# sksundaram-learning/linkerd

Measured on AMD Instinct MI355X. Metric: histogram samples ingested+summarized/sec (1M series) and % HBM peak, higher is better.
Workload: dtype u32; 1 GPU; C3: 1M series, 1e9 Zipf(s=1) samples per step, log-normal values; series_total=1000000, series_per_gpu=1000000, rotating_batches=3, parallelism=series-sharded x1 (weighted ranges), step=ingest (sample+plan+bin1+bin2) + snapshot(reset, dense counts + summaries)

## Files before the change

### linkerd_amd/csrc/l5dh_ingest.hip

```cpp
#include <algorithm>
#include <type_traits>

#include "l5dh_device.hpp"

namespace l5dh {
namespace {

constexpr uint32_t RSAMPLE = 1u << 18;
#ifndef L5DH_RS_WG
#define L5DH_RS_WG 64
#endif
constexpr int RS_WG = L5DH_RS_WG;
static_assert((RSAMPLE + RS_WG - 1) / RS_WG <= 65535, "k_rsample's u16 LDS counters: at most 65535 draws per workgroup");
constexpr uint32_t INVALID = 0xFFFFFFFFu;

__device__ __forceinline__ uint32_t round_up(uint32_t x, uint32_t m) { return (x + m - 1) / m * m; }

__device__ __forceinline__ uint32_t rcap(double prev, double e, double s, bool exact, double pad, uint32_t align,
                                         uint32_t pct, double z, bool floor_sample) {
  double c;
  if (exact) {
    c = e;
  } else {
    const double e0 = prev / s, sg = sqrt(e0 + 1.0);
    const double r = sqrt(e + 1.0) + 0.5 * z;
    const double sb = !floor_sample && prev == 0.0 && e == 0.0 ? ceil(4.0 * s) : ceil(r * r * s);
    if (prev > 0.0 && e >= e0 - 6.0 * sg && (floor_sample || e <= e0 + 4.0 * sg)) {
      c = ceil(prev * 1.0625 + 4.0 * sqrt(prev));
      if (floor_sample) c = fmax(c, sb);
    } else {
      c = sb;
    }
    c += pad;
  }
  if (pct != 100) c = floor(c * (double)pct / 100.0);
  return round_up((uint32_t)fmin(c, 1073741824.0), align);
}

__device__ __forceinline__ uint64_t block_excl_scan64(uint64_t v, uint64_t* lds , uint64_t* total) {
  const int lane = threadIdx.x & 63, w = threadIdx.x >> 6;
  const uint64_t incl = wave_incl_scan(v);
  if (lane == 63) lds[w] = incl;
  __syncthreads();
  if (threadIdx.x == 0) {
    uint64_t acc = 0;
    for (int k = 0; k < 16; ++k) {
      const uint64_t q = lds[k];
      lds[k] = acc;
      acc += q;
    }
    lds[16] = acc;
  }
  __syncthreads();
  const uint64_t r = lds[w] + incl - v;
  *total = lds[16];
  __syncthreads();
  return r;
}

#ifdef L5DH_PHASES
__device__ unsigned long long g_phase_plan[16];
#define RP_MARK(k) \
  if (threadIdx.x == 0) g_phase_plan[k] = wall_clock64();
#define RS_MARK(k) \
  if (threadIdx.x == 0 && blockIdx.x == 0) g_phase_plan[k] = wall_clock64();
#else
#define RP_MARK(k)
#define RS_MARK(k)
#endif

__global__ __launch_bounds__(1024) void k_rsample(const uint32_t* __restrict__ series, size_t n, uint32_t S, uint32_t K,
                                                  uint32_t* __restrict__ kest) {
  extern __shared__ uint32_t c[];
  RS_MARK(8)
  for (uint32_t i = threadIdx.x; i < (K + 1) / 2; i += 1024) c[i] = 0;
  __syncthreads();
  RS_MARK(9)
  const uint64_t m = n < RSAMPLE ? n : RSAMPLE;
  const uint64_t per = (m + RS_WG - 1) / RS_WG;
  const uint64_t k0 = blockIdx.x * per, k1 = k0 + per < m ? k0 + per : m;
  for (uint64_t kb = k0; kb < k1; kb += 4 * 1024) {
    uint32_t sv[4];
#pragma unroll
    for (int u = 0; u < 4; ++u) {
      const uint64_t k = kb + threadIdx.x + 1024u * u;
      const uint64_t i = m == n ? k : k * n / m;
      sv[u] = k < k1 ? series[i < n ? i : 0] : 0xFFFFFFFFu;
    }
#pragma unroll
    for (int u = 0; u < 4; ++u)
      if (sv[u] < S) {
        const uint32_t key = sv[u] >> 4;
        atomicAdd(&c[key >> 1], (key & 1u) ? 0x10000u : 1u);
      }
  }
  __syncthreads();
  RS_MARK(10)
  for (uint32_t i = threadIdx.x; i < (K + 1) / 2; i += 1024) {
    const uint32_t x = c[i];
    if (x & 0xFFFFu) atomicAdd(&kest[2 * i], x & 0xFFFFu);
    if ((x >> 16) && 2 * i + 1 < K) atomicAdd(&kest[2 * i + 1], x >> 16);
  }
  RS_MARK(11)
}

constexpr size_t RPLAN1_LDS = 32768 * 4;
constexpr uint32_t RFIX2_ONE_WG_MAX = 16384;
__global__ __launch_bounds__(1024) void k_rplan1(size_t n, uint32_t F, const uint32_t* __restrict__ kest,
                                                 const uint32_t* __restrict__ kprev, uint32_t* __restrict__ meta,
                                                 size_t cap32, size_t dlim16, uint32_t thr_min, uint32_t dmax,
                                                 uint32_t pct) {
  __shared__ uint32_t lh[33];
  __shared__ uint32_t sthr;
  __shared__ uint4 lds4[17];
  __shared__ uint64_t l64[17];
  __shared__ uint32_t dl[DIRECT_MAX + 1];
  __shared__ uint32_t capl[BIN1_BINS];
  extern __shared__ uint32_t tw[];
  const MetaLayout L = meta_layout(F);
  const uint32_t FS = (F + ST_TILES - 1) / ST_TILES;
  const uint32_t NW = (F + 31) / 32;
  const uint64_t m = n < RSAMPLE ? n : RSAMPLE;
  const bool exact = m == n;
  const double s = m ? (double)n / (double)m : 1.0;
  const uint32_t j = threadIdx.x, t0 = j * 32;
  const int lane = lane_id();
  RP_MARK(0)
  if (j < 33) lh[j] = 0;
  capl[j] = 0;
  auto load_pairs = [&](const uint32_t* __restrict__ kw, uint4 (&x)[16]) {
#pragma unroll
    for (int i = 0; i < 16; ++i) {
      const uint32_t t = 2u * (j + 1024u * (uint32_t)i);
      x[i] = make_uint4(0u, 0u, 0u, 0u);
      if (t + 1 < F) {
        x[i] = *reinterpret_cast<const uint4*>(kw + 2 * t);
      } else if (t < F) {
        x[i].x = kw[2 * t];
        x[i].y = kw[2 * t + 1];
      }
    }
  };
  uint2 te[16];
  {
    uint4 x[16];
    load_pairs(kest, x);
#pragma unroll
    for (int i = 0; i < 16; ++i) te[i] = make_uint2(x[i].x + x[i].y, x[i].z + x[i].w);
  }
  auto scaled = [&](uint32_t v) -> uint32_t { return (uint32_t)fmin((double)v * s, 4294967295.0); };
  __syncthreads();
  RP_MARK(1)
  auto hist = [&](uint32_t v) {
    const uint32_t e = scaled(v);
    const bool ok = dmax > 0 && e >= thr_min && e > 0;
    const int bin = ok ? 31 - __clz((int)e) : 0;
    const uint64_t act = __ballot(ok);
    if (!act) return;
    const int b0 = __builtin_amdgcn_readlane(bin, __builtin_ctzll(act));
    if (__ballot(ok && bin == b0) == act) {
      if (lane == 0) atomicAdd(&lh[b0], (uint32_t)__popcll(act));
    } else if (ok) {
      atomicAdd(&lh[bin], 1u);
    }
  };
#pragma unroll
  for (int i = 0; i < 16; ++i) {
    hist(te[i].x);
    hist(te[i].y);
  }
  __syncthreads();
  if (j < 64) {
    const uint32_t c = j < 32 ? lh[31 - j] : 0u;
    const uint32_t cum = wave_incl_scan32(c);
    const uint64_t ok = __ballot(dmax > 0 && j < 32 && cum <= dmax);
    const int nb = __popcll(ok);
    if (j == 0) sthr = nb ? max(max(thr_min, 1u), 1u << (32 - nb)) : 0xFFFFFFFFu;
  }
#pragma unroll
  for (int i = 0; i < 16; ++i) reinterpret_cast<uint2*>(tw)[j + 1024u * (uint32_t)i] = te[i];
  uint4 xp[16];
  load_pairs(kprev, xp);
  __syncthreads();
  const uint32_t thr = sthr;
  RP_MARK(2)
  uint32_t dbits = 0, E = 0;
#pragma unroll
  for (int k = 0; k < 32; ++k) {
    const uint32_t kk = (uint32_t)(k + (int)j) & 31u;
    const uint32_t v = tw[t0 + kk];
    if (t0 + kk < F && scaled(v) >= thr) dbits |= 1u << kk;
    else E += v;
  }
  __syncthreads();
#pragma unroll
  for (int i = 0; i < 16; ++i)
    reinterpret_cast<uint2*>(tw)[j + 1024u * (uint32_t)i] = make_uint2(xp[i].x + xp[i].y, xp[i].z + xp[i].w);
  __syncthreads();
  uint64_t P = 0;
#pragma unroll
  for (int k = 0; k < 32; ++k) {
    const uint32_t kk = (uint32_t)(k + (int)j) & 31u;
    if (!((dbits >> kk) & 1u)) P += tw[t0 + kk];
  }
  RP_MARK(3)
  uint32_t cv[4] = {(uint32_t)__popc(dbits), 0u, 0u, 0u}, ct[4];
  block_excl_scan4<1024>(cv, lds4, ct);
  const uint32_t ND = ct[0];
  meta[L.dbits() + j] = j < NW ? dbits : 0u;
  meta[L.dpre() + j] = cv[0];
  {
    uint32_t x = dbits, di = cv[0];
    while (x) {
      const uint32_t k = (uint32_t)(__ffs((int)x) - 1);
      x &= x - 1u;
      dl[di] = t0 + k;
      meta[L.dlist() + di] = t0 + k;
      ++di;
    }
  }
  P += __shfl_xor(P, 1, 64);
  E += __shfl_xor(E, 1, 64);
  RP_MARK(4)
  if ((j & 1u) == 0 && (j >> 1) < FS) {
    const uint32_t b = j >> 1;
    capl[b] = rcap((double)P, (double)E, s, exact, 256.0, 4, pct, 6.0, true);
    meta[L.btot() + b] = (uint32_t)min(P, (uint64_t)0xFFFFFFFFu);
  }
  __syncthreads();
  RP_MARK(5)
  const uint32_t TB = FS + 2 * ND;
  if (j >= FS && j < TB) {
    const uint32_t t = dl[(j - FS) >> 1], h = (j - FS) & 1u;
    const double p = (double)kprev[2 * t + h], e = (double)kest[2 * t + h];
    capl[j] = rcap(p, e, s, exact, 256.0, 8, pct, 5.0, false);
  }
  __syncthreads();
  const bool stb = j < FS, dj = j >= FS && j < TB;
  uint64_t tot32, tot16;
  const uint64_t base32 = block_excl_scan64(stb ? (uint64_t)capl[j] : 0ull, l64, &tot32);
  const uint64_t base16 = block_excl_scan64(dj ? (uint64_t)capl[j] : 0ull, l64, &tot16);
  const uint64_t base = stb ? base32 : base16;
  const uint64_t lim = stb ? cap32 : dlim16;
  if (base + capl[j] + 16 > lim)
    capl[j] = base + 16 < lim ? (uint32_t)(lim - 16 - base) & (stb ? ~3u : ~7u) : 0u;
  meta[L.bbase() + j] = (uint32_t)base;
  meta[L.bcap() + j] = j < TB ? capl[j] : 0u;
  meta[L.bcnt() + j] = 0u;
  if (j == 0) {
    uint32_t* hdr = meta + L.hdr();
    hdr[H_ND] = ND;
    hdr[H_OV1] = 0;
    hdr[H_REDO1] = 0;
    hdr[H_OV2] = 0;
    hdr[H_REDO2] = 0;
    hdr[H_COUNT2] = 0;
    hdr[H_EXACT] = exact ? 1u : 0u;
    hdr[H_D16] = (uint32_t)min(tot16, (uint64_t)dlim16);
  }
  RP_MARK(6)
}

#ifdef L5DH_PHASES
__device__ unsigned long long g_phase1[1024 * 8];
__device__ unsigned long long g_phase3[1024 * 8];
#define PH_INIT                                                            \
  const bool ph_on = threadIdx.x == 0 || threadIdx.x == NT1 - 64;          \
  uint32_t ph_acc[8] = {0, 0, 0, 0, 0, 0, 0, 0}, ph_t = (uint32_t)wall_clock64();
#define PH_VWAIT asm volatile("s_waitcnt vmcnt(0)" ::: "memory");
#define PH_MARK(k)                                 \
  if (ph_on) {                                     \
    const uint32_t ph_n = (uint32_t)wall_clock64(); \
    ph_acc[k] += ph_n - ph_t;                      \
    ph_t = ph_n;                                   \
  }
#define PH_FLUSH                                                                          \
  if (ph_on && pass == 0 && (threadIdx.x == 0 || gridDim.x <= 256)) {                      \
    const uint32_t ph_row = blockIdx.x + (threadIdx.x ? 512u : 0u);                       \
    for (int k = 0; k < 7; ++k) g_phase1[ph_row * 8 + k] += ph_acc[k];                    \
    g_phase1[ph_row * 8 + 7] += 1;                                                        \
    if (gridDim.x <= 256) {                                                               \
      g_phase1[(768 + blockIdx.x) * 8 + (threadIdx.x ? 1 : 0)] += ph_acc[7];              \
      if (threadIdx.x == 0) g_phase1[(768 + blockIdx.x) * 8 + 7] += 1;                    \
    }                                                                                     \
  }
#else
#define PH_INIT
#define PH_MARK(k)
#define PH_VWAIT
#define PH_FLUSH
#endif
__device__ __forceinline__ uint4 ld_stream(const uint32_t* p) { return *reinterpret_cast<const uint4*>(p); }
constexpr int CHW = 16384;
constexpr int NT1 = 1024;
constexpr int B1_PT = CHW / NT1;
constexpr int B1_PH = B1_PT / 2;
constexpr int B1_GS = 4;
constexpr int B1_HG = B1_PH / 4;
static_assert(B1_PH % 4 == 0 && B1_PH % B1_GS == 0 && B1_GS % 4 == 0, "halves of whole 16-B groups");
static_assert(NT1 == BIN1_BINS, "one bin per thread");
constexpr uint32_t DSUM_PMAX = 1u << 17;
static_assert(DSUM_PMAX == 1u << 17, "the ranking loop tests the bits of 2^17f, 0x48000000");
constexpr uint32_t NODEST = 0xFFFFFFFFu - (uint32_t)CHW;
constexpr int DSUM_N = DIRECT_MAX * TILE;

struct Bin1Lds {
  static constexpr int DW_N = 1024;
  static constexpr size_t o_stage = 0;
  static constexpr size_t o_cnt = o_stage + CHW * 4;
  static constexpr size_t o_offr = o_cnt + BIN1_BINS * 4;
  static constexpr size_t o_rdelta = o_offr + BIN1_BINS * 4;
  static constexpr size_t o_heads = o_rdelta + BIN1_BINS * 4;
  static constexpr size_t o_gpre = o_heads + CHW / 32 * 4;
  static constexpr size_t o_dw = o_gpre + CHW / 64 * 2;
  static constexpr size_t o_lut2 = o_dw + DW_N * 8;
  static constexpr size_t o_dsum = o_lut2 + LUT2_N * 8;
  static constexpr size_t o_dacc = o_dsum + DSUM_N * 4;
  static constexpr size_t o_breg = o_dacc + BIN1_BINS * 4;
  static constexpr size_t bytes = o_breg + BIN1_BINS * 8;

  template <typename T>
  static __device__ __forceinline__ T* at(uint32_t* smem, size_t o) {
    return reinterpret_cast<T*>(reinterpret_cast<char*>(smem) + o);
  }
  static __device__ __forceinline__ uint32_t* stage(uint32_t* smem) { return at<uint32_t>(smem, o_stage); }
  static __device__ __forceinline__ uint32_t* cnt(uint32_t* smem) { return at<uint32_t>(smem, o_cnt); }
  static __device__ __forceinline__ uint32_t* offr(uint32_t* smem) { return at<uint32_t>(smem, o_offr); }
  static __device__ __forceinline__ uint32_t* rdelta(uint32_t* smem) { return at<uint32_t>(smem, o_rdelta); }
  static __device__ __forceinline__ uint32_t* heads(uint32_t* smem) { return at<uint32_t>(smem, o_heads); }
  static __device__ __forceinline__ uint16_t* gpre(uint32_t* smem) { return at<uint16_t>(smem, o_gpre); }
  static __device__ __forceinline__ uint2* dw(uint32_t* smem) { return at<uint2>(smem, o_dw); }
  static __device__ __forceinline__ uint2* lut2(uint32_t* smem) { return at<uint2>(smem, o_lut2); }
  static __device__ __forceinline__ uint32_t* dsum(uint32_t* smem) { return at<uint32_t>(smem, o_dsum); }
  static __device__ __forceinline__ uint32_t* dacc(uint32_t* smem) { return at<uint32_t>(smem, o_dacc); }
  static __device__ __forceinline__ uint2* breg(uint32_t* smem) { return at<uint2>(smem, o_breg); }
};
static_assert(Bin1Lds::bytes <= 160 * 1024, "one workgroup's LDS");
static_assert(Bin1Lds::o_stage % 16 == 0 && Bin1Lds::o_heads % 16 == 0 && Bin1Lds::o_dw % 16 == 0 &&
                  Bin1Lds::o_lut2 % 16 == 0 && Bin1Lds::o_breg % 16 == 0,
              "stage and heads are accessed as uint4, dw, lut2 and breg as uint2");
static_assert(2ull * CHW * (DSUM_PMAX - 1) < (1ull << 32),
              "u32 direct sums: <= CHW (2^17 - 1) at a sub-chunk's start + as much from the sub-chunk");

static_assert(CHW <= 32768 && BIN1_BINS <= 1024, "15-bit ranks, 10-bit bins");
__device__ __forceinline__ uint32_t pk_make(uint32_t rank, uint32_t bin) { return rank | (bin << 15); }
__device__ __forceinline__ uint32_t pk_rank(uint32_t pk) { return pk & 0x7FFFu; }
__device__ __forceinline__ uint32_t pk_bin(uint32_t pk) { return (pk >> 15) & 1023u; }
static_assert(CHW < 65536, "16-bit stage offsets");
__device__ __forceinline__ uint32_t offr_make(uint32_t off, uint32_t run) { return off | (run << 16); }
__device__ __forceinline__ uint32_t offr_off(uint32_t w) { return w & 0xFFFFu; }
__device__ __forceinline__ uint32_t offr_run(uint32_t w) { return w >> 16; }

struct Bin1Run {
  uint32_t n, old;
  uint32_t base, cap;
};

__device__ __forceinline__ uint32_t b1_slot(uint32_t c0, int kk, int q) {
  return c0 + 4u * ((uint32_t)kk * NT1 + threadIdx.x) + (uint32_t)q;
}

struct Bin1Regs {
  uint4 s[B1_HG], v[B1_HG];
};
struct Bin1Half {
  uint32_t s[B1_PH];
  float f[B1_PH];
};

__device__ __forceinline__ Bin1Regs b1_issue_half(const uint32_t* series, const float* values, uint32_t c0, int h,
                                                  bool ok, const uint32_t* spare) {
  Bin1Regs r;
#pragma unroll
  for (int k = 0; k < B1_HG; ++k) {
    const uint32_t base = b1_slot(c0, h * B1_HG + k, 0);
    r.s[k] = ld_stream(ok ? series + base : spare);
    r.v[k] = ld_stream(ok ? reinterpret_cast<const uint32_t*>(values) + base : spare);
  }
  return r;
}
static_assert(B1_HG == 2 && B1_PH == 8, "the arrive points name a half's 16 registers");
__device__ __forceinline__ void b1_arrive(Bin1Regs& r) {
  asm volatile(""
               : "+v"(r.s[0].x), "+v"(r.s[0].y), "+v"(r.s[0].z), "+v"(r.s[0].w), "+v"(r.s[1].x), "+v"(r.s[1].y),
                 "+v"(r.s[1].z), "+v"(r.s[1].w), "+v"(r.v[0].x), "+v"(r.v[0].y), "+v"(r.v[0].z), "+v"(r.v[0].w),
                 "+v"(r.v[1].x), "+v"(r.v[1].y), "+v"(r.v[1].z), "+v"(r.v[1].w));
}
__device__ __forceinline__ void b1_arrive(Bin1Half& x) {
  asm volatile(""
               : "+v"(x.s[0]), "+v"(x.s[1]), "+v"(x.s[2]), "+v"(x.s[3]), "+v"(x.s[4]), "+v"(x.s[5]), "+v"(x.s[6]),
                 "+v"(x.s[7]), "+v"(x.f[0]), "+v"(x.f[1]), "+v"(x.f[2]), "+v"(x.f[3]), "+v"(x.f[4]), "+v"(x.f[5]),
                 "+v"(x.f[6]), "+v"(x.f[7]));
}

__device__ __forceinline__ Bin1Half b1_unpack_half(Bin1Regs r) {
  Bin1Half x;
#pragma unroll
  for (int k = 0; k < B1_HG; ++k) {
    const uint4 s4 = r.s[k], u4 = r.v[k];
    const float4 f4 = make_float4(__uint_as_float(u4.x), __uint_as_float(u4.y), __uint_as_float(u4.z),
                                  __uint_as_float(u4.w));
    x.s[4 * k] = s4.x; x.s[4 * k + 1] = s4.y; x.s[4 * k + 2] = s4.z; x.s[4 * k + 3] = s4.w;
    x.f[4 * k] = f4.x; x.f[4 * k + 1] = f4.y; x.f[4 * k + 2] = f4.z; x.f[4 * k + 3] = f4.w;
  }
  return x;
}
__device__ __forceinline__ Bin1Half b1_load_ragged(const uint32_t* series, const float* values, uint32_t c0,
                                                   uint32_t hi, int h) {
  Bin1Half x;
#pragma unroll
  for (int k = 0; k < B1_PH; ++k) {
    const uint32_t i = b1_slot(c0, h * B1_HG + (k >> 2), k & 3);
    const bool in = i < hi;
    x.s[k] = in ? series[i] : 0xFFFFFFFFu;
    x.f[k] = in ? values[i] : 0.0f;
  }
  return x;
}
__device__ __forceinline__ bool b1_ragged_invalid(Bin1Half x, uint32_t c0, uint32_t hi, int h, uint32_t S) {
  bool bad = false;
#pragma unroll
  for (int k = 0; k < B1_PH; ++k) bad |= b1_slot(c0, h * B1_HG + (k >> 2), k & 3) < hi && x.s[k] >= S;
  return bad;
}
__device__ __forceinline__ bool b1_group_invalid(Bin1Half x, int g, uint32_t S) {
  bool bad = false;
#pragma unroll
  for (int q = 0; q < B1_GS; ++q) bad |= x.s[g + q] >= S;
  return bad;
}

static_assert(B1_PT / B1_GS == 4, "one priority level per group of a sub-chunk");
__device__ __forceinline__ void b1_progress_prio(int gi) {
  if (gi == 0) __builtin_amdgcn_s_setprio(3);
  else if (gi == 1) __builtin_amdgcn_s_setprio(2);
  else if (gi == 2) __builtin_amdgcn_s_setprio(1);
  else __builtin_amdgcn_s_setprio(0);
}

static_assert(B1_GS == 4, "a group's pk words are returned as a uint4");
__device__ __forceinline__ uint4 b1_rank_group(uint32_t* smem, int h, int g, Bin1Half x, const uint32_t* series,
                                               const float* values, uint32_t c0, uint32_t S, uint32_t FS, uint32_t TB,
                                               Tables tb, int64_t* sumfix, int pass) {
  uint32_t* const stage = Bin1Lds::stage(smem);
  uint32_t* const cnt = Bin1Lds::cnt(smem);
  uint2* const dw = Bin1Lds::dw(smem);
  uint2* const lut2 = Bin1Lds::lut2(smem);
  uint32_t* const dsum = Bin1Lds::dsum(smem);
  constexpr int GS = B1_GS;
  uint32_t pl[GS], pk[GS];
  uint32_t escm = 0;
#pragma unroll
  for (int q = 0; q < GS; ++q) {
    const float f = x.f[g + q];
    const bool fast = __float_as_uint(f) < 0x48000000u;
    pl[q] = fast ? (uint32_t)f : 0u;
    escm |= (!fast && x.s[g + q] < S) ? (1u << q) : 0u;
  }
  if (__ballot(escm != 0u)) {
#pragma unroll 1
    for (int q = 0; q < GS; ++q) {
      if ((escm >> q) & 1u) {
        const uint32_t i = b1_slot(c0, h * B1_HG + (g + q) / 4, q & 3);
        uint32_t si = series[i];
        float vi = values[i];
        asm volatile("" : "+v"(si), "+v"(vi));
        const uint32_t r = payload1_slow(si, vi, tb, pass == 0 ? sumfix : nullptr);
        if (pass == 0 && r - DSUM_PMAX < V_ESC - DSUM_PMAX) {
          const uint2 d = dw[(si >> (TILE_SHIFT + 5)) & 1023u];
          if ((d.x >> ((si >> TILE_SHIFT) & 31u)) & 1u)
            atomicAdd(reinterpret_cast<unsigned long long*>(&sumfix[si]), (unsigned long long)r);
        }
#pragma unroll
        for (int u = 0; u < GS; ++u) pl[u] = q == u ? r : pl[u];
      }
    }
  }
  uint2 dv[GS], lv[GS];
#pragma unroll
  for (int q = 0; q < GS; ++q) dv[q] = dw[(x.s[g + q] >> (TILE_SHIFT + 5)) & 1023u];
#pragma unroll
  for (int q = 0; q < GS; ++q) lv[q] = lut2[lut2_index(pl[q])];
  uint32_t rc4[GS];
#pragma unroll
  for (int q = 0; q < GS; ++q) {
    const uint32_t s = x.s[g + q];
    const uint32_t tw = __builtin_amdgcn_ubfe(s, TILE_SHIFT, 5);
    const bool direct = s < S && __builtin_amdgcn_ubfe(dv[q].x, tw, 1) != 0u;
    const uint32_t di = dv[q].y + (uint32_t)__popc(__builtin_amdgcn_ubfe(dv[q].x, 0, tw));
    const uint32_t p = pl[q];
    uint32_t o;
    const uint32_t bk = lut2_decode(p, lv[q], o);
    const bool esc = p >= V_ESC;
    const uint32_t bucket = sel_u32(esc, p - V_ESC, bk);
    rc4[q] = sel_u32(direct, ((s & (TILE - 1)) << 11) | bucket, ((s & (ST_TILES * TILE - 1)) << 21) | p);
    const uint32_t dbin = FS + 2u * di + ((s >> 4) & 1u);
    const uint32_t bn = sel_u32(s < S, sel_u32(direct, dbin, s >> ST_SHIFT), TB);
    pk[q] = pk_make(atomicAdd(cnt + bn, 1u), bn);
    if (direct && pass == 0 && p - 1u < DSUM_PMAX - 1u) atomicAdd(&dsum[di * TILE + (s & (TILE - 1))], p);
  }
#pragma unroll
  for (int j = 0; j < GS / 4; ++j)
    *reinterpret_cast<uint4*>(stage + b1_slot(0u, h * B1_HG + g / 4 + j, 0)) =
        make_uint4(rc4[4 * j], rc4[4 * j + 1], rc4[4 * j + 2], rc4[4 * j + 3]);
  asm volatile("" ::: "memory");
  return make_uint4(pk[0], pk[1], pk[2], pk[3]);
}

__device__ __forceinline__ Bin1Run b1_reserve_run(uint32_t* smem, uint32_t tq, uint32_t TB, uint32_t* bcnt) {
  uint32_t* const cnt = Bin1Lds::cnt(smem);
  uint2* const breg = Bin1Lds::breg(smem);
  Bin1Run r;
  r.n = tq <= TB ? cnt[tq] : 0u;
  r.old = 0;
  const uint2 reg = breg[tq];
  r.base = reg.x;
  r.cap = reg.y;
  if (tq < TB && r.n) r.old = atomicAdd(&bcnt[tq], r.n);
  return r;
}

__device__ __forceinline__ void b1_guard_flush(uint32_t* smem, uint32_t tq, uint32_t rn, uint32_t FS, uint32_t TB,
                                               const uint32_t* meta, uint32_t dlist, uint32_t S, int64_t* sumfix) {
  uint32_t* const dsum = Bin1Lds::dsum(smem);
  uint32_t* const dacc = Bin1Lds::dacc(smem);
  bool fl = false;
  if (tq >= FS && tq < TB && rn) {
    const uint32_t A = dacc[tq] + rn;
    fl = A > (uint32_t)CHW;
    dacc[tq] = fl ? 0u : A;
  }
  for (uint64_t fm = __ballot(fl); fm; fm &= fm - 1) {
    const uint32_t fb = (tq & ~63u) + (uint32_t)__builtin_ctzll(fm) - FS;
    if ((tq & 63u) < TILE / 2) {
      const uint32_t h = fb * (TILE / 2) + (tq & 63u);
      const uint32_t v = dsum[h];
      dsum[h] = 0;
      const uint32_t sr = meta[dlist + h / TILE] * TILE + (h & (TILE - 1));
      if (v && sr < S) atomicAdd(reinterpret_cast<unsigned long long*>(&sumfix[sr]), (unsigned long long)v);
    }
  }
}

__device__ __forceinline__ uint32_t b1_scan_waves(uint32_t pv, uint32_t tq, uint32_t* wsum) {
  const uint32_t wi = wave_incl_scan32(pv);
  if ((tq & 63u) == 63u) wsum[tq >> 6] = wi;
  return wi;
}
__device__ __forceinline__ void b1_scan_heads(uint32_t* smem, const uint32_t* wsum, int wv, uint32_t pv, uint32_t wi,
                                              uint32_t rn) {
  uint32_t* const offr = Bin1Lds::offr(smem);
  uint32_t* const heads = Bin1Lds::heads(smem);
  uint32_t pre = 0;
  for (int q = 0; q < wv; ++q) pre += wsum[q];
  const uint32_t ex = pre + wi - pv;
  offr[threadIdx.x] = ex;
  if (rn) atomicOr(&heads[offr_off(ex) >> 5], 1u << (ex & 31u));
}

__device__ __forceinline__ void b1_read_slots(uint32_t* smem, uint32_t (&rec)[B1_PT]) {
  uint32_t* const stage = Bin1Lds::stage(smem);
#pragma unroll
  for (int kk = 0; kk < B1_PT / 4; ++kk) {
    const uint4 v = *reinterpret_cast<const uint4*>(stage + b1_slot(0u, kk, 0));
    rec[4 * kk] = v.x; rec[4 * kk + 1] = v.y; rec[4 * kk + 2] = v.z; rec[4 * kk + 3] = v.w;
  }
}

__device__ __forceinline__ void b1_scatter(uint32_t* smem, uint32_t pk, uint32_t rec) {
  uint32_t* const stage = Bin1Lds::stage(smem);
  uint32_t* const offr = Bin1Lds::offr(smem);
  stage[offr_off(offr[pk_bin(pk)]) + pk_rank(pk)] = rec;
}

__device__ __forceinline__ void b1_group_prefixes(uint32_t* smem, int lane) {
  uint32_t* const heads = Bin1Lds::heads(smem);
  uint16_t* const gpre = Bin1Lds::gpre(smem);
  constexpr int GPL = CHW / 64 / 64;
  static_assert(GPL % 2 == 0, "two groups per 16-B read");
  uint32_t pc[GPL], t = 0;
#pragma unroll
  for (int k = 0; k < GPL; k += 2) {
    const uint4 w = *reinterpret_cast<const uint4*>(heads + 2u * (GPL * (uint32_t)lane + (uint32_t)k));
    pc[k] = (uint32_t)(__popc(w.x) + __popc(w.y));
    pc[k + 1] = (uint32_t)(__popc(w.z) + __popc(w.w));
    t += pc[k] + pc[k + 1];
  }
  uint32_t ex = wave_incl_scan32(t) - t;
#pragma unroll
  for (int k = 0; k < GPL; ++k) {
    gpre[GPL * (uint32_t)lane + (uint32_t)k] = (uint16_t)ex;
    ex += pc[k];
  }
}

__device__ __forceinline__ void b1_run_delta(uint32_t* smem, const Bin1Run& r, uint32_t TB, uint32_t* hdr) {
  uint32_t* const offr = Bin1Lds::offr(smem);
  uint32_t* const rdelta = Bin1Lds::rdelta(smem);
  const uint32_t b = threadIdx.x;
  if (r.n) {
    uint32_t d = NODEST;
    if (b < TB) {
      if (r.old + r.n <= r.cap) d = r.base + r.old - offr_off(offr[b]);
      else hdr[H_OV1] = 1u;
    }
    rdelta[offr_run(offr[b])] = d;
  }
}

__device__ __forceinline__ void b1_write_out(uint32_t* smem, int wv, int lane, uint32_t nst, uint32_t* rec32,
                                             uint16_t* rec16) {
  uint32_t* const stage = Bin1Lds::stage(smem);
  uint32_t* const rdelta = Bin1Lds::rdelta(smem);
  uint32_t* const heads = Bin1Lds::heads(smem);
  uint16_t* const gpre = Bin1Lds::gpre(smem);
#pragma unroll 4
  for (int k = 0; k < B1_PT; ++k) {
    const uint32_t i = (uint32_t)wv * (B1_PT * 64) + (uint32_t)k * 64 + (uint32_t)lane;
    const uint32_t g = i >> 6;
    const unsigned long long hw = *reinterpret_cast<const unsigned long long*>(heads + 2 * g);
    const uint32_t run = (uint32_t)gpre[g] + mask_below(hw) + (uint32_t)((hw >> lane) & 1ull) - 1u;
    const uint32_t d = rdelta[run];
    if (d != NODEST) {
      if (run < nst)
        rec32[i + d] = stage[i];
      else
        rec16[i + d] = (uint16_t)stage[i];
    }
  }
}

__device__ __forceinline__ void b1_flush_sums(uint32_t* smem, uint32_t ND, const uint32_t* dlist, uint32_t S,
                                              int64_t* sumfix) {
  uint32_t* const dsum = Bin1Lds::dsum(smem);
  for (uint32_t i = threadIdx.x; i < ND * TILE; i += NT1) {
    const unsigned long long v = dsum[i];
    const uint32_t s = dlist[i / TILE] * TILE + (i & (TILE - 1));
    if (v && s < S) atomicAdd(reinterpret_cast<unsigned long long*>(&sumfix[s]), (unsigned long long)v);
  }
}

__global__ __launch_bounds__(NT1) void k_rbin1w(const uint32_t* __restrict__ series, const float* __restrict__ values,
                                                size_t n, size_t per, uint32_t S, uint32_t F, Tables tb,
                                                uint32_t* __restrict__ meta, uint32_t* __restrict__ rec32,
                                                uint16_t* __restrict__ rec16, int64_t* __restrict__ sumfix,
                                                uint32_t* __restrict__ err, int vec, int pass) {
  extern __shared__ __attribute__((aligned(16))) uint32_t smem[];
  __shared__ uint32_t wsum[NT1 / 64];
  uint32_t* const cnt = Bin1Lds::cnt(smem);
  uint32_t* const offr = Bin1Lds::offr(smem);
  uint32_t* const heads = Bin1Lds::heads(smem);
  uint2* const dw = Bin1Lds::dw(smem);
  uint2* const lut2 = Bin1Lds::lut2(smem);
  uint32_t* const dsum = Bin1Lds::dsum(smem);
  uint32_t* const dacc = Bin1Lds::dacc(smem);
  uint2* const breg = Bin1Lds::breg(smem);
  const MetaLayout L = meta_layout(F);
  uint32_t* hdr = meta + L.hdr();
  if (pass == 1 && __builtin_amdgcn_readfirstlane(hdr[H_REDO1]) == 0u) return;
  uint32_t* bcnt = meta + L.bcnt();
  const uint32_t* bbase = meta + L.bbase();
  const uint32_t* bcap = meta + L.bcap();
  const uint32_t* dlist = meta + L.dlist();
  const uint32_t FS = (F + ST_TILES - 1) / ST_TILES;
  const uint32_t NW = (F + 31) / 32;
  const uint32_t ND = hdr[H_ND];
  const uint32_t TB = FS + 2 * ND;
  const int lane = lane_id();
  const int wv = threadIdx.x >> 6;
  for (uint32_t w = threadIdx.x; w < NW; w += NT1) dw[w] = make_uint2(meta[L.dbits() + w], meta[L.dpre() + w]);
  cnt[threadIdx.x] = 0;
  dacc[threadIdx.x] = 0;
  for (uint32_t i = threadIdx.x; i < LUT2_N; i += NT1) lut2[i] = tb.lut2[i];
  for (uint32_t i = threadIdx.x; i < ND * TILE; i += NT1) dsum[i] = 0;
  __syncthreads();
  const uint32_t lo = (uint32_t)((size_t)blockIdx.x * per);
  const uint32_t hi = (uint32_t)min((size_t)lo + per, n);
  bool bad = false;
  {
    const uint32_t b = threadIdx.x;
    breg[b] = b < TB ? make_uint2(bbase[b], bcap[b]) : make_uint2(0u, 0u);
  }
  PH_INIT
  const uint32_t* const spare = reinterpret_cast<const uint32_t*>(tb.lim_pad);
  Bin1Regs pf = b1_issue_half(series, values, lo, 0, vec && lo + (uint32_t)CHW <= hi, spare);
  b1_arrive(pf);
  for (uint32_t c0 = lo; c0 < hi; c0 += CHW) {
    for (uint32_t wd = threadIdx.x; wd < CHW / 32; wd += NT1) heads[wd] = 0u;
    uint32_t pk[B1_PT];
    const bool full = vec && c0 + (uint32_t)CHW <= hi;
    Bin1Regs sh;
#pragma unroll
    for (int h = 0; h < 2; ++h) {
      if (h == 1) { PH_MARK(1) }
      Bin1Half hf;
      if (full) {
        hf = b1_unpack_half(h == 0 ? pf : sh);
      } else {
        hf = b1_load_ragged(series, values, c0, hi, h);
        b1_arrive(hf);
        bad |= b1_ragged_invalid(hf, c0, hi, h, S);
      }
      if (full) {
        PH_VWAIT
        if (h == 0) { PH_MARK(0) } else { PH_MARK(2) }
      }
#pragma unroll
      for (int g = 0; g < B1_PH; g += B1_GS) {
        if (h == 0 && g == B1_GS) sh = b1_issue_half(series, values, c0, 1, full, spare);
        if (h == 1 && g == B1_PH - B1_GS)
          pf = b1_issue_half(series, values, c0 + (uint32_t)CHW, 0, vec && c0 + 2u * (uint32_t)CHW <= hi, spare);
        b1_progress_prio(h * (B1_PH / B1_GS) + g / B1_GS);
        if (full) bad |= b1_group_invalid(hf, g, S);
        const uint4 p4 = b1_rank_group(smem, h, g, hf, series, values, c0, S, FS, TB, tb, sumfix, pass);
        pk[h * B1_PH + g] = p4.x; pk[h * B1_PH + g + 1] = p4.y; pk[h * B1_PH + g + 2] = p4.z; pk[h * B1_PH + g + 3] = p4.w;
      }
    }
    PH_MARK(3)
    __syncthreads();
    PH_MARK(7)
    uint32_t tq = threadIdx.x;
    asm volatile("" : "+v"(tq));
    const Bin1Run run = b1_reserve_run(smem, tq, TB, bcnt);
    if (pass == 0) b1_guard_flush(smem, tq, run.n, FS, TB, meta, L.dlist(), S, sumfix);
    const uint32_t pv = offr_make(run.n, run.n ? 1u : 0u);
    const uint32_t wi = b1_scan_waves(pv, tq, wsum);
    __syncthreads();
    b1_scan_heads(smem, wsum, wv, pv, wi, run.n);
    uint32_t rec[B1_PT];
    b1_read_slots(smem, rec);
    __syncthreads();
    PH_MARK(4)
#pragma unroll
    for (int k = 0; k < B1_PT; ++k) b1_scatter(smem, pk[k], rec[k]);
    if (wv == 0) b1_group_prefixes(smem, lane);
    b1_run_delta(smem, run, TB, hdr);
    __syncthreads();
    PH_MARK(5)
    const uint32_t nst = offr_run(offr[FS]);
    cnt[threadIdx.x] = 0;
    b1_arrive(pf);
    b1_write_out(smem, wv, lane, nst, rec32, rec16);
    __syncthreads();
    PH_MARK(6)
  }
  PH_FLUSH
  if (pass == 0) {
    b1_flush_sums(smem, ND, dlist, S, sumfix);
    if (bad) atomicAdd(err, 1u);
  }
}

__device__ __forceinline__ uint32_t lut3_byte(uint32_t v) {
  const uint32_t sh = 25u - (uint32_t)__builtin_clz(v | 64u);
  return ((v >> sh) + (sh << 6)) << 3;
}
__device__ __forceinline__ uint32_t lut3_bucket(uint32_t v, uint2 x) {
  return (x.x & 0x7FFu) + (((v << 11) | 0x7FFu) >= x.x ? 1u : 0u) + (v >= x.y ? 1u : 0u);
}

__global__ __launch_bounds__(1024) void k_rfix1(uint32_t F, uint32_t* __restrict__ meta, const uint32_t* __restrict__ err,
                                                uint32_t* __restrict__ err_host) {
  __shared__ uint32_t lds[17];
  const MetaLayout L = meta_layout(F);
  uint32_t* hdr = meta + L.hdr();
  if (threadIdx.x == 0) *reinterpret_cast<volatile uint32_t*>(err_host) = *err;
  const uint32_t FS = (F + ST_TILES - 1) / ST_TILES;
  const uint32_t ND = hdr[H_ND];
  const uint32_t TB = FS + 2 * ND;
  const uint32_t ov = hdr[H_OV1];
  const uint32_t b = threadIdx.x;
  const bool stb = b < FS, dj = b >= FS && b < TB;
  const uint32_t c = b < TB ? meta[L.bcnt() + b] : 0u;
  if (stb && !hdr[H_EXACT]) {
    const double P = (double)meta[L.btot() + b];
    if ((double)c > P * 1.0625 + 4.0 * sqrt(P) + 256.0) hdr[H_COUNT2] = 1u;
  }
  meta[L.btot() + b] = c;
  uint32_t t32, t16;
  const uint32_t nb32 = block_excl_scan<1024>(stb ? round_up(c, 4) : 0u, lds, &t32);
  const uint32_t nb16 = block_excl_scan<1024>(dj ? round_up(c, 8) : 0u, lds, &t16);
  const uint32_t nb = stb ? nb32 : nb16;
  const uint32_t base = ov ? nb : meta[L.bbase() + b];
  if (dj) {
    const uint32_t t = meta[L.dlist() + ((b - FS) >> 1)], h = (b - FS) & 1u;
    meta[L.kbase() + 2 * t + h] = base;
    meta[L.kcnt() + 2 * t + h] = c;
  }
  if (ov) {
    meta[L.bbase() + b] = nb;
    meta[L.bcap() + b] = round_up(c, stb ? 4 : 8);
    meta[L.bcnt() + b] = 0u;
  }
  const uint32_t d16 = hdr[H_D16];
  if (ov && t16 > d16) {
    for (uint32_t k = b; k < L.K; k += 1024)
      if (!((meta[L.dbits() + (k >> 6)] >> ((k >> 1) & 31u)) & 1u)) meta[L.kcap() + k] = 0u;
  }
  uint32_t all;
  const uint32_t is = block_excl_scan<1024>(stb ? (c + ITEM2 - 1) / ITEM2 : 0u, lds, &all);
  if (stb) meta[L.istart() + b] = is;
  __syncthreads();
  if (b == 0) {
    meta[L.istart() + FS] = all;
    hdr[H_ITEMS] = all;
    if (ov && t16 > d16) {
      hdr[H_D16] = t16;
      hdr[H_COUNT2] = 1u;
    }
    hdr[H_OV2] = 0u;
    hdr[H_REDO2] = 0u;
    hdr[H_REDO1] = ov;
    hdr[H_OV1] = 0u;
    if (ov) hdr[H_NOVR1] += 1u;
  }
}

__device__ __forceinline__ bool tile_direct(const uint32_t* __restrict__ meta, const MetaLayout& L, uint32_t t) {
  return (meta[L.dbits() + (t >> 5)] >> (t & 31u)) & 1u;
}

__device__ __forceinline__ uint64_t wsum_before(const uint64_t* __restrict__ ws, uint32_t b, uint64_t* red ) {
  uint64_t v = threadIdx.x < b ? ws[threadIdx.x] : 0ull;
  v = wave_sum(v);
  if ((threadIdx.x & 63) == 0) red[threadIdx.x >> 6] = v;
  __syncthreads();
  uint64_t r = 0;
  for (int q = 0; q < 16; ++q) r += red[q];
  __syncthreads();
  return r;
}

__global__ __launch_bounds__(1024) void k_rplan2a(size_t n, uint32_t F, uint32_t* __restrict__ kest,
                                                  const uint32_t* __restrict__ kprev, uint32_t* __restrict__ meta,
                                                  uint32_t pct) {
  __shared__ uint64_t red[16];
  const MetaLayout L = meta_layout(F);
  const uint64_t m = n < RSAMPLE ? n : RSAMPLE;
  const bool exact = m == n;
  const double s = m ? (double)n / (double)m : 1.0;
  const uint32_t k = blockIdx.x * 1024u + threadIdx.x;
  uint32_t cap = 0;
  if (k < L.K) {
    const uint32_t e = kest[k];
    if (e) kest[k] = 0;
    if (!tile_direct(meta, L, k >> 1)) {
      cap = rcap((double)kprev[k], (double)e, s, exact, 32.0, 8, pct, 5.0, false);
      meta[L.kcap() + k] = cap;
    }
  }
  const uint64_t w = wave_sum((uint64_t)cap);
  if ((threadIdx.x & 63) == 0) red[threadIdx.x >> 6] = w;
  __syncthreads();
  if (threadIdx.x == 0) {
    uint64_t t = 0;
    for (int q = 0; q < 16; ++q) t += red[q];
    reinterpret_cast<uint64_t*>(meta + L.wsum())[blockIdx.x] = t;
  }
}

__global__ __launch_bounds__(1024) void k_rplan2b(uint32_t F, uint32_t* __restrict__ meta, size_t cap16) {
  __shared__ uint64_t red[16];
  __shared__ uint64_t l64[17];
  const MetaLayout L = meta_layout(F);
  uint32_t* hdr = meta + L.hdr();
  const uint64_t before = wsum_before(reinterpret_cast<const uint64_t*>(meta + L.wsum()), blockIdx.x, red);
  const uint32_t k = blockIdx.x * 1024u + threadIdx.x;
  const bool mine = k < L.K && !tile_direct(meta, L, k >> 1);
  uint32_t cap = mine ? meta[L.kcap() + k] : 0u;
  uint64_t total;
  const uint64_t base = hdr[H_D16] + before + block_excl_scan64((uint64_t)cap, l64, &total);
  if (mine) {
    if (base + cap + 64 > cap16) {
      cap = base + 64 < cap16 ? (uint32_t)(cap16 - 64 - base) & ~7u : 0u;
      hdr[H_COUNT2] = 1u;
    }
    meta[L.kbase() + k] = (uint32_t)base;
    meta[L.kcap() + k] = cap;
    meta[L.kcnt() + k] = 0u;
  }
}

constexpr int B2_KEYS = 2 * ST_TILES;
constexpr int B2_NT = 512, B2_PER_CU = 2;
constexpr size_t rbin2_lds() {
  return 2048 * 8 + LUT2_N * 8 + 2 * B2_KEYS * 8 + (B2_KEYS + 64) * 4 + 2 * (size_t)ITEM2 * 4;
}

template <int NT>
__global__ __launch_bounds__(NT, B2_PER_CU * NT / 256) void k_rbin2(uint32_t S, uint32_t F, Tables tb, uint32_t* __restrict__ meta,
                                                 const uint32_t* __restrict__ m_is, const uint32_t* __restrict__ m_bb,
                                                 const uint32_t* __restrict__ m_bt,
                                                 const uint32_t* __restrict__ rec32, uint16_t* __restrict__ rec16,
                                                 int64_t* __restrict__ sumfix, int pass) {
  constexpr int PT = (int)ITEM2 / NT;
  constexpr int PG = PT / 4;
  __shared__ __attribute__((aligned(16))) uint32_t smem[rbin2_lds() / 4];
  unsigned long long* lsum = reinterpret_cast<unsigned long long*>(smem);
  uint2* lut3 = reinterpret_cast<uint2*>(lsum + 2048);
  uint2* ocx = lut3 + LUT2_N;
  uint32_t* cnt = reinterpret_cast<uint32_t*>(ocx + 2 * B2_KEYS);
  uint32_t* stage = cnt + B2_KEYS + 64;
  const MetaLayout L = meta_layout(F);
  uint32_t* hdr = meta + L.hdr();
  if (pass == 1 && __builtin_amdgcn_readfirstlane(hdr[H_REDO2]) == 0u) return;
  const uint32_t nitems = hdr[H_ITEMS];
  const uint32_t i0 = (uint32_t)(((uint64_t)blockIdx.x * nitems) / gridDim.x);
  const uint32_t i1 = (uint32_t)(((uint64_t)(blockIdx.x + 1) * nitems) / gridDim.x);
  if (i0 >= i1) return;
  const uint32_t FS = (F + ST_TILES - 1) / ST_TILES;
  uint32_t* kcnt = meta + L.kcnt();
  const uint32_t* kbase = meta + L.kbase();
  const uint32_t* kcap = meta + L.kcap();
  const int lane = lane_id(), wv = threadIdx.x >> 6;
  for (int i = threadIdx.x; i < LUT2_N; i += NT) lut3[i] = tb.lut3[i];
  for (int i = threadIdx.x; i < 2048; i += NT) lsum[i] = 0ull;
  for (int i = threadIdx.x; i < B2_KEYS; i += NT) cnt[i] = 0u;
  uint32_t jl = 0, jh = FS;
  while (jh - jl > 1) {
    const uint32_t mid = (jl + jh) >> 1;
    if (m_is[mid] <= i0) jl = mid; else jh = mid;
  }
  __syncthreads();
  uint32_t jn = jl;
  auto item_range = [&](uint32_t item, uint32_t& j, uint32_t& a, uint32_t& e) {
    while (m_is[jn + 1] <= item) jn = __builtin_amdgcn_readfirstlane(jn + 1);
    j = jn;
    const uint32_t bb = m_bb[jn];
    a = bb + (item - m_is[jn]) * ITEM2;
    e = min(a + ITEM2, bb + m_bt[jn]);
  };
  auto load = [&](uint32_t a, uint32_t e, uint4 (&x)[PG]) {
#pragma unroll
    for (int g = 0; g < PG; ++g) {
      const uint32_t idx = a + 4u * ((uint32_t)g * NT + threadIdx.x);
      x[g] = *reinterpret_cast<const uint4*>(rec32 + (idx < e ? idx : a));
    }
  };
  uint32_t cur_j = 0xFFFFFFFFu;
  auto flush = [&](uint32_t jj) {
    for (int i = threadIdx.x; i < 2048; i += NT) {
      const unsigned long long v = lsum[i];
      const uint32_t s = jj * 2048u + (uint32_t)i;
      if (v && s < S) atomicAdd(reinterpret_cast<unsigned long long*>(&sumfix[s]), v);
      lsum[i] = 0ull;
    }
  };
  if (pass == 0 && __builtin_amdgcn_readfirstlane(hdr[H_COUNT2]) != 0u) {
    uint32_t j, a, e;
    item_range(i0, j, a, e);
    uint4 x[PG];
    load(a, e, x);
    for (uint32_t item = i0; item < i1; ++item) {
      const uint32_t cj = j, ctot = e - a;
      uint4 xn[PG];
      if (item + 1 < i1) item_range(item + 1, j, a, e);
      load(a, e, xn);
      if (cj != cur_j) {
        if (cur_j != 0xFFFFFFFFu) {
          __syncthreads();
          flush(cur_j);
        }
        cur_j = cj;
        __syncthreads();
      }
#pragma unroll
      for (int g = 0; g < PG; ++g) {
        const uint32_t rr[4] = {x[g].x, x[g].y, x[g].z, x[g].w};
#pragma unroll
        for (int q = 0; q < 4; ++q) {
          const uint32_t p = rr[q] & 0x1FFFFFu;
          const bool valid = 4u * ((uint32_t)g * NT + threadIdx.x) + (uint32_t)q < ctot;
          atomicAdd(&cnt[valid ? rr[q] >> 25 : (uint32_t)B2_KEYS + (uint32_t)lane], 1u);
          atomicAdd(&lsum[(rr[q] >> 21) & 2047u], (unsigned long long)((valid && p < V_ESC) ? p : 0u));
        }
      }
      __syncthreads();
      if (wv < 2) {
        const uint32_t rk = (uint32_t)wv * 64u + (uint32_t)lane;
        const uint32_t rc = cnt[rk];
        if (rc) atomicAdd(&kcnt[cj * (uint32_t)B2_KEYS + rk], rc);
        cnt[rk] = 0u;
      }
      __syncthreads();
#pragma unroll
      for (int g = 0; g < PG; ++g) x[g] = xn[g];
    }
    __syncthreads();
    flush(cur_j);
    return;
  }
  auto write_out = [&](int bb, uint32_t total) {
    const uint32_t* st = stage + bb * ITEM2;
    const uint2* oc = ocx + bb * B2_KEYS;
    constexpr int WB = 4;
#pragma unroll
    for (int k0 = 0; k0 < PT; k0 += WB) {
      uint32_t x[WB];
      uint2 o[WB];
#pragma unroll
      for (int j = 0; j < WB; ++j) x[j] = st[(uint32_t)wv * (PT * 64) + (uint32_t)(k0 + j) * 64 + (uint32_t)lane];
#pragma unroll
      for (int j = 0; j < WB; ++j) o[j] = oc[(x[j] >> 16) & (B2_KEYS - 1)];
#pragma unroll
      for (int j = 0; j < WB; ++j) {
        const uint32_t i = (uint32_t)wv * (PT * 64) + (uint32_t)(k0 + j) * 64 + (uint32_t)lane;
        if (i < total && o[j].y != INVALID) rec16[o[j].y + (i - o[j].x)] = (uint16_t)(x[j] & 0xFFFFu);
      }
      __builtin_amdgcn_sched_barrier(0);
    }
  };
  uint32_t j, a, e;
  item_range(i0, j, a, e);
  uint4 x[PG];
  load(a, e, x);
  uint32_t prev_total = 0;
#ifdef L5DH_PHASES
  unsigned long long ph2[5] = {0, 0, 0, 0, 0}, ph2_t = wall_clock64();
#define PH2_MARK(k)                                  \
  if (threadIdx.x == 0) {                            \
    const unsigned long long ph_n = wall_clock64();  \
    ph2[k] += ph_n - ph2_t;                          \
    ph2_t = ph_n;                                    \
  }
#else
#define PH2_MARK(k)
#endif
// ... 298 lines not shown
```

Before: 186.0 billion samples/s.

## Grow bin1 chunk to three parts and move per-bin state into registers

Each bin1 workgroup now handles its chunk as B1_NP parts of 8 samples per thread, 3 by default, so CHW grows from 16K to 24K slots. The aim is to amortize the per-chunk barriers, scan, atomic reservation and write-out over more samples. The per-bin dacc and breg arrays move out of LDS into registers, which frees the LDS the larger stage buffer needs. The direct-sum flush threshold is re-derived to keep u32 sums from overflowing, and a 6-level progress-priority table is added. The cost is more live registers per thread (24 pk plus the rec words), which may spill or lower occupancy, and LDS is now within a few hundred bytes of the limit.

```diff
diff --git a/linkerd_amd/csrc/l5dh_ingest.hip b/linkerd_amd/csrc/l5dh_ingest.hip
--- a/linkerd_amd/csrc/l5dh_ingest.hip
+++ b/linkerd_amd/csrc/l5dh_ingest.hip
@@ -291,16 +291,25 @@
 #define PH_FLUSH
 #endif
 __device__ __forceinline__ uint4 ld_stream(const uint32_t* p) { return *reinterpret_cast<const uint4*>(p); }
-constexpr int CHW = 16384;
+#ifndef L5DH_B1_NP
+#define L5DH_B1_NP 3
+#endif
 constexpr int NT1 = 1024;
-constexpr int B1_PT = CHW / NT1;
-constexpr int B1_PH = B1_PT / 2;
+constexpr int B1_NP = L5DH_B1_NP;
+constexpr int B1_PH = 8;
+constexpr int B1_PT = B1_NP * B1_PH;
+constexpr int CHW = B1_PT * NT1;
 constexpr int B1_GS = 4;
 constexpr int B1_HG = B1_PH / 4;
-static_assert(B1_PH % 4 == 0 && B1_PH % B1_GS == 0 && B1_GS % 4 == 0, "halves of whole 16-B groups");
+static_assert(B1_NP == 2 || B1_NP == 3, "the progress priorities are written out for 4 and 6 groups");
+static_assert(B1_PH % 4 == 0 && B1_PH % B1_GS == 0 && B1_GS % 4 == 0, "parts of whole 16-B groups");
 static_assert(NT1 == BIN1_BINS, "one bin per thread");
 constexpr uint32_t DSUM_PMAX = 1u << 17;
 static_assert(DSUM_PMAX == 1u << 17, "the ranking loop tests the bits of 2^17f, 0x48000000");
+constexpr uint32_t DSUM_FLUSH = 32768u - (uint32_t)CHW;
+static_assert(CHW < 32768, "a flush bound above 0");
+static_assert((uint64_t)(DSUM_FLUSH + (uint32_t)CHW) * (DSUM_PMAX - 1) < (1ull << 32),
+              "u32 direct sums: <= DSUM_FLUSH (2^17 - 1) at a sub-chunk's start + CHW (2^17 - 1) from the sub-chunk");
 constexpr uint32_t NODEST = 0xFFFFFFFFu - (uint32_t)CHW;
 constexpr int DSUM_N = DIRECT_MAX * TILE;
 
@@ -315,9 +324,8 @@
   static constexpr size_t o_dw = o_gpre + CHW / 64 * 2;
   static constexpr size_t o_lut2 = o_dw + DW_N * 8;
   static constexpr size_t o_dsum = o_lut2 + LUT2_N * 8;
-  static constexpr size_t o_dacc = o_dsum + DSUM_N * 4;
-  static constexpr size_t o_breg = o_dacc + BIN1_BINS * 4;
-  static constexpr size_t bytes = o_breg + BIN1_BINS * 8;
+  static constexpr size_t bytes = o_dsum + DSUM_N * 4;
+  static constexpr size_t static_bytes = NT1 / 64 * 4;
 
   template <typename T>
   static __device__ __forceinline__ T* at(uint32_t* smem, size_t o) {
@@ -332,15 +340,12 @@
   static __device__ __forceinline__ uint2* dw(uint32_t* smem) { return at<uint2>(smem, o_dw); }
   static __device__ __forceinline__ uint2* lut2(uint32_t* smem) { return at<uint2>(smem, o_lut2); }
   static __device__ __forceinline__ uint32_t* dsum(uint32_t* smem) { return at<uint32_t>(smem, o_dsum); }
-  static __device__ __forceinline__ uint32_t* dacc(uint32_t* smem) { return at<uint32_t>(smem, o_dacc); }
-  static __device__ __forceinline__ uint2* breg(uint32_t* smem) { return at<uint2>(smem, o_breg); }
 };
-static_assert(Bin1Lds::bytes <= 160 * 1024, "one workgroup's LDS");
+static_assert(Bin1Lds::bytes + Bin1Lds::static_bytes <= 160 * 1024, "one workgroup's LDS");
+static_assert(B1_NP != 3 || Bin1Lds::bytes == 163456, "24 K slots: 384 B short of the 160 KB");
 static_assert(Bin1Lds::o_stage % 16 == 0 && Bin1Lds::o_heads % 16 == 0 && Bin1Lds::o_dw % 16 == 0 &&
-                  Bin1Lds::o_lut2 % 16 == 0 && Bin1Lds::o_breg % 16 == 0,
-              "stage and heads are accessed as uint4, dw, lut2 and breg as uint2");
-static_assert(2ull * CHW * (DSUM_PMAX - 1) < (1ull << 32),
-              "u32 direct sums: <= CHW (2^17 - 1) at a sub-chunk's start + as much from the sub-chunk");
+                  Bin1Lds::o_lut2 % 16 == 0,
+              "stage and heads are accessed as uint4, dw and lut2 as uint2");
 
 static_assert(CHW <= 32768 && BIN1_BINS <= 1024, "15-bit ranks, 10-bit bins");
 __device__ __forceinline__ uint32_t pk_make(uint32_t rank, uint32_t bin) { return rank | (bin << 15); }
@@ -430,11 +435,16 @@
   return bad;
 }
 
-static_assert(B1_PT / B1_GS == 4, "one priority level per group of a sub-chunk");
+#ifndef L5DH_B1_PRIO6
+#define L5DH_B1_PRIO6 3, 3, 2, 2, 1, 0
+#endif
 __device__ __forceinline__ void b1_progress_prio(int gi) {
-  if (gi == 0) __builtin_amdgcn_s_setprio(3);
-  else if (gi == 1) __builtin_amdgcn_s_setprio(2);
-  else if (gi == 2) __builtin_amdgcn_s_setprio(1);
+  constexpr int lv4[4] = {3, 2, 1, 0}, lv6[6] = {L5DH_B1_PRIO6};
+  static_assert(B1_PT / B1_GS == 4 || B1_PT / B1_GS == 6, "a priority level per group of a sub-chunk");
+  const int p = B1_PT / B1_GS == 4 ? lv4[gi & 3] : lv6[gi];
+  if (p == 3) __builtin_amdgcn_s_setprio(3);
+  else if (p == 2) __builtin_amdgcn_s_setprio(2);
+  else if (p == 1) __builtin_amdgcn_s_setprio(1);
   else __builtin_amdgcn_s_setprio(0);
 }
 
@@ -507,13 +517,12 @@
   return make_uint4(pk[0], pk[1], pk[2], pk[3]);
 }
 
-__device__ __forceinline__ Bin1Run b1_reserve_run(uint32_t* smem, uint32_t tq, uint32_t TB, uint32_t* bcnt) {
+__device__ __forceinline__ Bin1Run b1_reserve_run(uint32_t* smem, uint32_t tq, uint32_t TB, uint32_t* bcnt,
+                                                  uint2 reg) {
   uint32_t* const cnt = Bin1Lds::cnt(smem);
-  uint2* const breg = Bin1Lds::breg(smem);
   Bin1Run r;
   r.n = tq <= TB ? cnt[tq] : 0u;
   r.old = 0;
-  const uint2 reg = breg[tq];
   r.base = reg.x;
   r.cap = reg.y;
   if (tq < TB && r.n) r.old = atomicAdd(&bcnt[tq], r.n);
@@ -521,14 +530,14 @@
 }
 
 __device__ __forceinline__ void b1_guard_flush(uint32_t* smem, uint32_t tq, uint32_t rn, uint32_t FS, uint32_t TB,
-                                               const uint32_t* meta, uint32_t dlist, uint32_t S, int64_t* sumfix) {
+                                               const uint32_t* meta, uint32_t dlist, uint32_t S, int64_t* sumfix,
+                                               uint32_t& dacc) {
   uint32_t* const dsum = Bin1Lds::dsum(smem);
-  uint32_t* const dacc = Bin1Lds::dacc(smem);
   bool fl = false;
   if (tq >= FS && tq < TB && rn) {
-    const uint32_t A = dacc[tq] + rn;
-    fl = A > (uint32_t)CHW;
-    dacc[tq] = fl ? 0u : A;
+    const uint32_t A = dacc + rn;
+    fl = A > DSUM_FLUSH;
+    dacc = fl ? 0u : A;
   }
   for (uint64_t fm = __ballot(fl); fm; fm &= fm - 1) {
     const uint32_t fb = (tq & ~63u) + (uint32_t)__builtin_ctzll(fm) - FS;
@@ -653,8 +662,6 @@
   uint2* const dw = Bin1Lds::dw(smem);
   uint2* const lut2 = Bin1Lds::lut2(smem);
   uint32_t* const dsum = Bin1Lds::dsum(smem);
-  uint32_t* const dacc = Bin1Lds::dacc(smem);
-  uint2* const breg = Bin1Lds::breg(smem);
   const MetaLayout L = meta_layout(F);
   uint32_t* hdr = meta + L.hdr();
   if (pass == 1 && __builtin_amdgcn_readfirstlane(hdr[H_REDO1]) == 0u) return;
@@ -670,17 +677,14 @@
   const int wv = threadIdx.x >> 6;
   for (uint32_t w = threadIdx.x; w < NW; w += NT1) dw[w] = make_uint2(meta[L.dbits() + w], meta[L.dpre() + w]);
   cnt[threadIdx.x] = 0;
-  dacc[threadIdx.x] = 0;
   for (uint32_t i = threadIdx.x; i < LUT2_N; i += NT1) lut2[i] = tb.lut2[i];
   for (uint32_t i = threadIdx.x; i < ND * TILE; i += NT1) dsum[i] = 0;
   __syncthreads();
   const uint32_t lo = (uint32_t)((size_t)blockIdx.x * per);
   const uint32_t hi = (uint32_t)min((size_t)lo + per, n);
   bool bad = false;
-  {
-    const uint32_t b = threadIdx.x;
-    breg[b] = b < TB ? make_uint2(bbase[b], bcap[b]) : make_uint2(0u, 0u);
-  }
+  const uint2 breg = threadIdx.x < TB ? make_uint2(bbase[threadIdx.x], bcap[threadIdx.x]) : make_uint2(0u, 0u);
+  uint32_t dacc = 0;
   PH_INIT
   const uint32_t* const spare = reinterpret_cast<const uint32_t*>(tb.lim_pad);
   Bin1Regs pf = b1_issue_half(series, values, lo, 0, vec && lo + (uint32_t)CHW <= hi, spare);
@@ -691,8 +695,8 @@
     const bool full = vec && c0 + (uint32_t)CHW <= hi;
     Bin1Regs sh;
 #pragma unroll
-    for (int h = 0; h < 2; ++h) {
-      if (h == 1) { PH_MARK(1) }
+    for (int h = 0; h < B1_NP; ++h) {
+      if (h >= 1) { PH_MARK(1) }
       Bin1Half hf;
       if (full) {
         hf = b1_unpack_half(h == 0 ? pf : sh);
@@ -707,8 +711,8 @@
       }
 #pragma unroll
       for (int g = 0; g < B1_PH; g += B1_GS) {
-        if (h == 0 && g == B1_GS) sh = b1_issue_half(series, values, c0, 1, full, spare);
-        if (h == 1 && g == B1_PH - B1_GS)
+        if (h + 1 < B1_NP && g == B1_GS) sh = b1_issue_half(series, values, c0, h + 1, full, spare);
+        if (h == B1_NP - 1 && g == B1_PH - B1_GS)
           pf = b1_issue_half(series, values, c0 + (uint32_t)CHW, 0, vec && c0 + 2u * (uint32_t)CHW <= hi, spare);
         b1_progress_prio(h * (B1_PH / B1_GS) + g / B1_GS);
         if (full) bad |= b1_group_invalid(hf, g, S);
@@ -721,8 +725,8 @@
     PH_MARK(7)
     uint32_t tq = threadIdx.x;
     asm volatile("" : "+v"(tq));
-    const Bin1Run run = b1_reserve_run(smem, tq, TB, bcnt);
-    if (pass == 0) b1_guard_flush(smem, tq, run.n, FS, TB, meta, L.dlist(), S, sumfix);
+    const Bin1Run run = b1_reserve_run(smem, tq, TB, bcnt, breg);
+    if (pass == 0) b1_guard_flush(smem, tq, run.n, FS, TB, meta, L.dlist(), S, sumfix, dacc);
     const uint32_t pv = offr_make(run.n, run.n ? 1u : 0u);
     const uint32_t wi = b1_scan_waves(pv, tq, wsum);
     __syncthreads();
```

After: 183.8 billion samples/s. 1.2% lower.
